# MengLing-L/distributed_plonk

Measured on AMD Instinct MI355X. Metric: constraints/sec = n / proof time (verified five-round proof, dispatcher2.rs:192-713; BN254 PLONK), higher is better.
Workload: dtype u32x8 Montgomery (256-bit Fr/Fq)

## Files before the change

distributed_plonk_amd/csrc/ntt_engine.hip:

```cpp
#include <algorithm>
#include <cstdlib>
#include <cstring>

#include "constants.h"
#include "ntt_kernels.hpp"
#include "plonk_internal.hpp"

static int ilog2(uint64_t x) { int l = 0; while (((uint64_t)1 << (l + 1)) <= x) l++; return l; }
static_assert(NTT_LOG_RMAX == 9, "NttTables::max_log_r defaults to NTT_LOG_RMAX");

const FrParams& fr_params(int curve) { return curve == PLONK_BN254 ? BN254_FR_PARAMS : BLS12_381_FR_PARAMS; }

static Fr host_pow2k(const Fr& a, int k, const FrParams& P) {
    Fr r = a;
    for (int i = 0; i < k; i++) r = fp_sqr(r, P);
    return r;
}

static int upload_powers(F29** d_out, const Fr& base, size_t count, const Fr& first, const FrParams& P, hipStream_t stream) {
    std::vector<F29> h(count);
    Fr r261;
    for (int i = 0; i < 8; i++) r261.l[i] = P.one[i];
    for (int i = 0; i < 5; i++) r261 = fp_add(r261, r261, P);
    const Fr k_mont = fp_to_mont(r261, P);
// ... 33 lines not shown
        if ((rc = upload_powers(&T.tw_small[d], host_pow2k(w[d], T.two_adicity - NTT_LOG_RMAX, P),
                                (size_t)1 << (NTT_LOG_RMAX - 1), one, P, stream))) return rc;
        {
            const size_t cnt = (size_t)1 << (NTT_LOG_RMAX - 1);
            std::vector<F29S> h(cnt);
            const Fr base = host_pow2k(w[d], T.two_adicity - NTT_LOG_RMAX, P);
            Fr acc = one;
            for (size_t i = 0; i < cnt; i++) { h[i] = f29_shoup_from_mont256(acc, P); acc = fp_mul(acc, base, P); }
            HIP_TRY(hipMalloc((void**)&T.tw_shoup[d], cnt * sizeof(F29S)));
            HIP_TRY(hipMemcpyAsync(T.tw_shoup[d], h.data(), cnt * sizeof(F29S), hipMemcpyHostToDevice, stream));
            HIP_TRY(hipStreamSynchronize(stream));
        }
        if ((rc = upload_powers(&T.g_lo[d], g[d], nt, one, P, stream))) return rc;
        if ((rc = upload_powers(&T.g_hi[d], host_pow2k(g[d], T.lt, P), nt, one, P, stream))) return rc;
    }
    T.use_shoup = getenv("PLONK_NTT_NO_SHOUP") == nullptr;
    Fr two = fp_add(one, one, P), half = fp_inv(two, P);
    T.h_pow2_inv.resize(T.two_adicity + 1);
    Fr acc = one;
    for (int k = 0; k <= T.two_adicity; k++) { T.h_pow2_inv[k] = acc; acc = fp_mul(acc, half, P); }
    return PLONK_OK;
}

void ntt_tables_trim(NttTables& T) {
    for (auto& kv : T.tw_lo_scaled) (void)hipFree(kv.second);
    T.tw_lo_scaled.clear();
    for (auto& kv : T.planes) (void)hipFree(kv.second);
    T.planes.clear();
    for (auto& kv : T.rowtabs) (void)hipFree(kv.second);
    T.rowtabs.clear();
    for (auto& kv : T.shift_sets) { (void)hipFree(kv.second.planes); (void)hipFree(kv.second.rowtabs); (void)hipFree(kv.second.foldc); }
    T.shift_sets.clear();
    T.plane_bytes = 0;
    for (auto& kv : T.quot_inv_xm1) (void)hipFree(kv.second);
    T.quot_inv_xm1.clear();
    for (auto& kv : T.pow_tabs) (void)hipFree(kv.second);
    T.pow_tabs.clear();
    T.pow_order.clear();
}

void ntt_tables_destroy(NttTables& T) {
    for (int d = 0; d < 2; d++) {
        (void)hipFree(T.tw_shoup[d]); T.tw_shoup[d] = nullptr;
        (void)hipFree(T.tw_small[d]); (void)hipFree(T.tw_lo[d]); (void)hipFree(T.tw_hi[d]); (void)hipFree(T.g_lo[d]); (void)hipFree(T.g_hi[d]);
        T.tw_small[d] = T.tw_lo[d] = T.tw_hi[d] = T.g_lo[d] = T.g_hi[d] = nullptr;
    }
    for (auto& kv : T.tw_lo_scaled) (void)hipFree(kv.second);
    T.tw_lo_scaled.clear();
    for (auto& kv : T.planes) (void)hipFree(kv.second);
    T.planes.clear();
    for (auto& kv : T.rowtabs) (void)hipFree(kv.second);
    T.rowtabs.clear();
    for (auto& kv : T.shift_sets) { (void)hipFree(kv.second.planes); (void)hipFree(kv.second.rowtabs); (void)hipFree(kv.second.foldc); }
    T.shift_sets.clear();
    T.plane_bytes = 0;
    if (T.quot_x_lo) { (void)hipFree(T.quot_x_lo); T.quot_x_lo = nullptr; }
    for (auto& kv : T.quot_inv_xm1) (void)hipFree(kv.second);
    T.quot_inv_xm1.clear();
    for (auto& kv : T.pow_tabs) (void)hipFree(kv.second);
    T.pow_tabs.clear();
    T.pow_order.clear();
}

static int get_scaled_lo(NttTables& T, int log_m, F29** out, hipStream_t stream) {
    auto it = T.tw_lo_scaled.find(log_m);
    if (it != T.tw_lo_scaled.end()) { *out = it->second; return PLONK_OK; }
    F29* d = nullptr;
    int rc = upload_powers(&d, T.h_root[1], (size_t)1 << T.lt, T.h_pow2_inv[log_m], T.fp, stream);
    if (rc) return rc;
    T.tw_lo_scaled[log_m] = d;
    *out = d;
    return PLONK_OK;
}

static void plane_fallback_notice(const char* why, size_t bytes) {
    static bool said = false;
// ... 53 lines not shown
    hipError_t e = hipGetLastError();
    if (e != hipSuccess) { (void)hipFree(d); return plonk_fail(PLONK_ERR_HIP, "ntt_gen_epi_plane launch: %s", hipGetErrorString(e)); }
    T.planes[key] = d;
    T.plane_bytes += bytes;
    *out = d;
    return PLONK_OK;
}

static int get_rowtab(NttTables& T, int log_r1, int log_w, F29** out, hipStream_t stream) {
    const uint64_t key = ((uint64_t)log_r1 << 8) | (uint64_t)log_w;
    auto it = T.rowtabs.find(key);
    if (it != T.rowtabs.end()) { *out = it->second; return PLONK_OK; }
    const uint32_t* g_l = T.curve == PLONK_BN254 ? BN254_FR_GENERATOR_MONT : BLS12_381_FR_GENERATOR_MONT;
    Fr base = fp_from_limbs<8>(g_l);
    for (int i = 0; i < log_r1; i++) base = fp_sqr(base, T.fp);
    F29* d = nullptr;
    int rc = upload_powers(&d, base, (size_t)1 << log_w, fp_one(T.fp), T.fp, stream);
    if (rc) return rc;
    T.rowtabs[key] = d;
    *out = d;
    return PLONK_OK;
}

static void host_powers_const(std::vector<F29>& h, const Fr& base, size_t count, const FrParams& P) {
    Fr r261;
    for (int i = 0; i < 8; i++) r261.l[i] = P.one[i];
    for (int i = 0; i < 5; i++) r261 = fp_add(r261, r261, P);
    const Fr k_mont = fp_to_mont(r261, P);
    Fr acc = fp_one(P);
    for (size_t i = 0; i < count; i++) {
        h.push_back(f29_from_sat(fp_from_mont(fp_mul(acc, k_mont, P), P)));
        acc = fp_mul(acc, base, P);
    }
}

static int get_shift_set(NttTables& T, const Fr& h, int L, uint64_t B, int w0, int NP, const NttTables::ShiftSet** out, hipStream_t stream) {
    const FrParams& P = T.fp;
    const int logB = ilog2(B);
    std::string key((const char*)h.l, 32);
    key.push_back((char)L); key.push_back((char)logB); key.push_back((char)w0);
    auto it = T.shift_sets.find(key);
    if (it != T.shift_sets.end()) { *out = &it->second; return PLONK_OK; }
    if (L + logB > T.two_adicity) return plonk_fail(PLONK_ERR_DOMAIN, "coset classes: 2^%d points exceed the two-adicity", L + logB);
    const uint64_t M = (uint64_t)1 << L, R1 = (uint64_t)1 << w0, r1 = M >> w0;
    NttTables::ShiftSet set;
    set.bytes = NP > 1 ? (size_t)(B * M) * sizeof(Fr) : 0;
    if (T.plane_bytes + set.bytes > T.plane_budget && !T.shift_sets.empty()) {
        HIP_TRY(hipStreamSynchronize(stream));
        for (auto& kv : T.shift_sets) {
            (void)hipFree(kv.second.planes); (void)hipFree(kv.second.rowtabs); (void)hipFree(kv.second.foldc);
            T.plane_bytes -= kv.second.bytes;
        }
        T.shift_sets.clear();
    }
    if (T.plane_bytes + set.bytes > T.plane_budget)
        return plonk_fail(PLONK_ERR_HIP, "coset classes: %zu bytes of first-pass planes exceed the plane budget (%zu of %zu in use)", set.bytes,
                          T.plane_bytes, T.plane_budget);
    const Fr wB = host_pow2k(T.h_root[0], T.two_adicity - (L + logB), P);
    std::vector<F29> h_row, h_fold;
    h_row.reserve(B * R1); h_fold.reserve(B * NTT_MAX_FOLD);
    std::vector<Fr> hq(B);
    Fr acc = h;
    for (uint64_t q = 0; q < B; q++) { hq[q] = acc; acc = fp_mul(acc, wB, P); }
    for (uint64_t q = 0; q < B; q++) {
        host_powers_const(h_row, host_pow2k(hq[q], L - w0, P), R1, P);
        host_powers_const(h_fold, host_pow2k(hq[q], L, P), NTT_MAX_FOLD, P);
    }
    struct Guard {
        NttTables::ShiftSet* s; F29* extra = nullptr; bool armed = true;
        ~Guard() { if (armed) { (void)hipFree(s->planes); (void)hipFree(s->rowtabs); (void)hipFree(s->foldc); } (void)hipFree(extra); }
    } guard{&set};
    HIP_TRY(hipMalloc((void**)&set.rowtabs, h_row.size() * sizeof(F29)));
    HIP_TRY(hipMalloc((void**)&set.foldc, h_fold.size() * sizeof(F29)));
    HIP_TRY(hipMemcpyAsync(set.rowtabs, h_row.data(), h_row.size() * sizeof(F29), hipMemcpyHostToDevice, stream));
    HIP_TRY(hipMemcpyAsync(set.foldc, h_fold.data(), h_fold.size() * sizeof(F29), hipMemcpyHostToDevice, stream));
    HIP_TRY(hipStreamSynchronize(stream));
    if (NP > 1) {
        if (hipMalloc((void**)&set.planes, set.bytes) != hipSuccess) {
            (void)hipGetLastError();
            set.planes = nullptr;
            return plonk_fail(PLONK_ERR_HIP, "coset classes: out of memory for %zu bytes of first-pass planes", set.bytes);
        }
        const size_t n_hi = (size_t)std::max<uint64_t>(1, r1 >> 10);
        std::vector<F29> h_pw;
        h_pw.reserve(B * (1024 + n_hi));
        for (uint64_t q = 0; q < B; q++) {
            host_powers_const(h_pw, hq[q], 1024, P);
            host_powers_const(h_pw, host_pow2k(hq[q], 10, P), n_hi, P);
        }
        F29* d_pw = nullptr;
        HIP_TRY(hipMalloc((void**)&d_pw, h_pw.size() * sizeof(F29)));
        guard.extra = d_pw;
        HIP_TRY(hipMemcpyAsync(d_pw, h_pw.data(), h_pw.size() * sizeof(F29), hipMemcpyHostToDevice, stream));
        for (uint64_t q = 0; q < B; q++) {
            const F29* lo = d_pw + q * (1024 + n_hi);
            ProfScope ps("ntt_gen_shift_plane", stream);
            hipLaunchKernelGGL(ntt_gen_shift_plane_kernel, dim3((uint32_t)((M + 255) / 256)), dim3(256), 0, stream, set.planes + q * M, M, r1, T.tw_lo[0],
                               T.tw_hi[0], (uint32_t)T.lt, (uint32_t)(T.two_adicity - L), lo, lo + 1024, T.fp29);
// ... 44 lines not shown
    if (s.kind == 1 || s.kind == 2) {
        o.lo = T.g_lo[s.kind - 1];
        o.hi = T.g_hi[s.kind - 1];
    } else {
        const int d = s.kind - 3;
        o.lo = T.tw_lo[d];
        o.hi = T.tw_hi[d];
        const int sh = T.two_adicity - s.log_order;
        aq <<= sh; a0 <<= sh; bq <<= sh; b0 <<= sh;
    }
    o.aq = aq; o.a0 = a0; o.bq = bq; o.b0 = b0;
    return o;
}

static int ntt_ept() {
    static const int ept = [] {
        const char* e = getenv("PLONK_NTT_EPT");
        const int v = e ? atoi(e) : 4;
        return (v == 4 || v == 2) ? v : (e ? 8 : 4);
    }();
    return ept;
}

template <int LOG_R, int EPT, bool SWZ = false, bool SHOUP = false>
static hipError_t launch_one_e(const NttPassParams& P, uint64_t grid, uint32_t threads, size_t lds, hipStream_t stream) {
    static DeviceOnce attr;
    hipError_t e = attr.run([] { return hipFuncSetAttribute(reinterpret_cast<const void*>(&ntt_pass_kernel<LOG_R, EPT, SWZ, SHOUP>),
                                                           hipFuncAttributeMaxDynamicSharedMemorySize, 160 * 1024); });
    if (e != hipSuccess) return e;
    hipLaunchKernelGGL((ntt_pass_kernel<LOG_R, EPT, SWZ, SHOUP>), dim3((uint32_t)grid), dim3(threads), lds, stream, P);
    return hipGetLastError();
}
static bool swizzle_on() {
    static const bool on = getenv("PLONK_NTT_NO_SWIZZLE") == nullptr;
    return on;
}
template <int LOG_R>
static hipError_t launch_one(const NttPassParams& P, uint64_t grid, uint32_t threads, size_t lds, hipStream_t stream) {
    if constexpr (LOG_R >= 5) {
        if (ntt_ept() == 4 && P.log_t == 3 && P.tile_pitch == 8 && swizzle_on()) {
            if (P.tw_shoup != nullptr) return launch_one_e<LOG_R, 4, true, true>(P, grid, threads, lds, stream);
            return launch_one_e<LOG_R, 4, true>(P, grid, threads, lds, stream);
        }
    }
    if (ntt_ept() == 4) return launch_one_e<LOG_R, 4>(P, grid, threads, lds, stream);
    if (ntt_ept() == 2) return launch_one_e<LOG_R, 2>(P, grid, threads, lds, stream);
    return launch_one_e<LOG_R, 8>(P, grid, threads, lds, stream);
}

static hipError_t launch_pass(int log_r, const NttPassParams& P, uint64_t grid, uint32_t threads, size_t lds, hipStream_t s) {
    switch (log_r) {
        case 1: return launch_one<1>(P, grid, threads, lds, s);
        case 2: return launch_one<2>(P, grid, threads, lds, s);
        case 3: return launch_one<3>(P, grid, threads, lds, s);
        case 4: return launch_one<4>(P, grid, threads, lds, s);
        case 5: return launch_one<5>(P, grid, threads, lds, s);
        case 6: return launch_one<6>(P, grid, threads, lds, s);
        case 7: return launch_one<7>(P, grid, threads, lds, s);
        case 8: return launch_one<8>(P, grid, threads, lds, s);
        case 9: return launch_one<9>(P, grid, threads, lds, s);
    }
    return hipErrorInvalidValue;
}
// ... 109 lines not shown
                P.plane_rp = r_p;
            }
            avail = interleaved ? Bt : r_p;
            int lt = std::min(pref_log_t(w), ilog2(avail));
            const uint64_t Tt = (uint64_t)1 << lt;
            P.log_t = lt;
            if (!interleaved) {
                P.n0 = r_p / Tt; P.n1 = M / r_prev;
                P.ls0 = Tt; P.ls1 = r_prev; P.ls2 = M; P.l_astride = r_p; P.l_tstride = 1;
                P.bs0 = Tt; P.bs1 = 0; P.tb = 1;
                P.qs0 = 0; P.qs1 = 0; P.qs2 = 1; P.tq = 0;
                P.pa = r_p; P.ps0 = Tt; P.ps1 = 0; P.pt = 1;
                grid = Bt * P.n1 * P.n0;
            } else {
                P.n0 = Bt / Tt; P.n1 = r_p;
                P.ls0 = Tt; P.ls1 = Bt; P.ls2 = r_prev * Bt; P.l_astride = r_p * Bt; P.l_tstride = 1;
                P.bs0 = 0; P.bs1 = 1; P.tb = 0;
                P.qs0 = Tt; P.qs1 = 0; P.qs2 = 0; P.tq = 1;
                P.pa = r_p; P.ps0 = 0; P.ps1 = 1; P.pt = 0;
                grid = (M / r_prev) * P.n1 * P.n0;
            }
            P.ss0 = P.ls0; P.ss1 = P.ls1; P.ss2 = P.ls2; P.s_istride = P.l_astride; P.s_tstride = 1;
            P.tile_pitch = (uint32_t)Tt;
        } else {
            P.out = c.out;
            P.kstride = M >> w;
            if (sset != nullptr && NP >= 2 && n_cls >= 2) {
                avail = Bt;
                int lt = std::min(pref_log_t(w), ilog2(avail));
                const uint64_t Tt = (uint64_t)1 << lt;
                P.log_t = lt;
                P.n0 = Bt / Tt; P.n1 = M >> w;
                P.ls0 = Tt * M; P.ls1 = R; P.ls2 = 0; P.l_astride = 1; P.l_tstride = M; P.load_a_fast = 1;
                P.qs0 = Tt; P.tq = 1;
                P.ms0 = 0; P.tk = 0;
                P.rev_ndig = NP - 1;
                for (int d = 0; d < NP - 1; d++) P.rev_w[d] = widths[d];
                P.rev_shift0 = 0;
                grid = P.n0 * P.n1;
            } else if (!interleaved && NP >= 2) {
                const uint64_t R1 = (uint64_t)1 << widths[0], r1 = M >> widths[0];
                avail = R1;
                int lt = std::min(pref_log_t(w), ilog2(avail));
                const uint64_t Tt = (uint64_t)1 << lt;
                P.log_t = lt;
                P.n0 = R1 / Tt; P.n1 = (M >> w) / R1;
// ... 37 lines not shown
            if (c.inverse && NP == 1) { P.scale_const_enabled = 1; P.scale_const = f29_const_from_mont256(T.h_pow2_inv[L], T.fp); }
            if (epi_plane != nullptr && (!need_q_const || coset_folded || sset != nullptr)) {
                P.epi_plane = epi_plane;
                P.epi_qstride = M * n_cls;
            } else {
                P.epi = make_scale(T, c.epi, c.q_offset);
            }
            P.tile_pitch = (uint32_t)((uint64_t)1 << P.log_t);
        }
        if (p == 0 && !coset_folded) P.pro = make_scale(T, c.pro, c.q_offset);
        const uint64_t Tt = (uint64_t)1 << P.log_t;
        const uint32_t ept = (R >= (uint64_t)ntt_ept()) ? (uint32_t)ntt_ept() : (uint32_t)R;
        const uint32_t threads = (uint32_t)(R * Tt / ept);
        if (threads > 1024) return plonk_fail(PLONK_ERR_ARG, "ntt_run: tile of %llu x %llu needs %u lanes", (unsigned long long)R, (unsigned long long)Tt, threads);
        const size_t lds = (size_t)9 * R * P.tile_pitch * 4 + std::max<size_t>(R / 2, 1) * 36;
        if (grid == 0 || grid > 0x7fffffffull) return plonk_fail(PLONK_ERR_ARG, "ntt_run: grid %llu out of range", (unsigned long long)grid);
        static const char* const kNames[10] = {"", "ntt_pass_kernel<1>", "ntt_pass_kernel<2>", "ntt_pass_kernel<3>", "ntt_pass_kernel<4>",
                                               "ntt_pass_kernel<5>", "ntt_pass_kernel<6>", "ntt_pass_kernel<7>", "ntt_pass_kernel<8>",
                                               "ntt_pass_kernel<9>"};
        hipError_t e;
        {
            ProfScope ps_all("ntt_pass_kernel", stream);
            ProfScope ps_w(kNames[w], stream);
            e = launch_pass(w, P, grid, threads, lds, stream);
        }
        if (e != hipSuccess) return plonk_fail(PLONK_ERR_HIP, "ntt pass launch (log_r=%d, grid=%llu, threads=%u, lds=%zu): %s", w,
                                               (unsigned long long)grid, threads, lds, hipGetErrorString(e));
        r_prev = r_p;
    }
    return PLONK_OK;
}

__global__ void __launch_bounds__(256) transpose_fr_kernel(const Fr* __restrict__ in, Fr* __restrict__ out, uint64_t rows, uint64_t cols) {
    __shared__ uint4 tile[16][16 * 2 + 1];
    const uint64_t tiles_c = (cols + 15) / 16;
    const uint64_t tr = blockIdx.x / tiles_c, tc = blockIdx.x % tiles_c;
    const uint32_t ly = threadIdx.x / 16, lx = threadIdx.x % 16;
    uint64_t r = tr * 16 + ly, cc = tc * 16 + lx;
    if (r < rows && cc < cols) {
        const uint4* src = reinterpret_cast<const uint4*>(in + r * cols + cc);
        tile[ly][2 * lx] = src[0];
        tile[ly][2 * lx + 1] = src[1];
    }
    __syncthreads();
    uint64_t orow = tc * 16 + ly, ocol = tr * 16 + lx;
    if (orow < cols && ocol < rows) {
// ... 17 lines not shown
```

distributed_plonk_amd/csrc/ntt_kernels.hpp:

```cpp
#pragma once
#include "fp.hpp"
#include "fp29.hpp"

typedef Fp<8> Fr;
typedef FpParams<8> FrParams;

#define NTT_LOG_RMAX 9
#define NTT_MAX_PASSES 4
#define NTT_MAX_FOLD 8

struct TwoLevelScale {
    const F29* lo;
    const F29* hi;
    uint64_t aq, a0, bq, b0;
    uint32_t lt;
    uint32_t enabled;
};

struct NttPassParams {
    const Fr* in;
    Fr* out;
    F29Params fp;
    const F29* tw_small;
    const F29S* tw_shoup;
// ... 17 lines not shown
    uint32_t rev_ndig;
    uint32_t rev_w[NTT_MAX_PASSES];
    uint32_t rev_shift0;
    uint64_t oq, ok;
    int32_t split_log;
    uint64_t split_blk;
    const Fr* tw_plane;
    uint64_t plane_rp;
    const F29* pro_rowtab;
    uint64_t rowtab_qstride;
    uint64_t plane_qstride;
    uint64_t in_len;
    uint64_t fold_m;
    uint32_t nfold;
    const F29* fold_c;
    uint32_t cls_log;
    uint64_t in_row_pitch;
    const Fr* epi_plane;
    uint64_t epi_qstride;
    uint32_t scale_const_enabled;
    F29 scale_const;
    TwoLevelScale pro;
    TwoLevelScale epi;
};

__device__ __forceinline__ Fr load_fr(const Fr* p) {
    const uint4* q = reinterpret_cast<const uint4*>(p);
    uint4 a = q[0], b = q[1];
    Fr r;
    r.l[0] = a.x; r.l[1] = a.y; r.l[2] = a.z; r.l[3] = a.w;
    r.l[4] = b.x; r.l[5] = b.y; r.l[6] = b.z; r.l[7] = b.w;
    return r;
}
__device__ __forceinline__ void store_fr(Fr* p, const Fr& v) {
    uint4* q = reinterpret_cast<uint4*>(p);
    q[0] = make_uint4(v.l[0], v.l[1], v.l[2], v.l[3]);
    q[1] = make_uint4(v.l[4], v.l[5], v.l[6], v.l[7]);
}
__device__ __forceinline__ F29 load_f29(const F29* p) {
    F29 r;
    const uint32_t* q = reinterpret_cast<const uint32_t*>(p);
#pragma unroll
    for (int i = 0; i < 9; i++) r.l[i] = q[i];
    return r;
}
__device__ __forceinline__ F29 params_one(const F29Params& P) {
// ... 25 lines not shown
    __device__ __forceinline__ void put(uint32_t idx, const F29& v) const {
#pragma unroll
        for (int l = 0; l < 9; l++) base[l * plane + idx] = v.l[l];
    }
};

template <bool SWZ> __device__ __forceinline__ uint32_t sw_fold(uint32_t row) {
    if (!SWZ) return 0;
    uint32_t y = row >> 2;
    y ^= y >> 4;
    y ^= y >> 2;
    return y & 3;
}

template <int LOG_R>
__device__ __forceinline__ void shoup_tw_load(const F29S* __restrict__ tab, uint32_t e, uint32_t* cw) {
    const uint4* src = reinterpret_cast<const uint4*>(tab + ((size_t)e << (NTT_LOG_RMAX - LOG_R)));
#pragma unroll
    for (int j = 0; j < 5; j++) {
        const uint4 d = src[j];
        cw[4 * j] = d.x; cw[4 * j + 1] = d.y; cw[4 * j + 2] = d.z; cw[4 * j + 3] = d.w;
    }
}
template <int LOG_R, int K, bool FIRST, bool SHOUP>
__device__ __forceinline__ void ntt_butterflies(F29 (&v)[1 << K], int s0, uint32_t lo, const uint32_t* tw_lds, const F29S* __restrict__ tw_shoup,
                                                const F29Params& fp) {
    constexpr int R = 1 << LOG_R;
    constexpr int RADIX = 1 << K;
    constexpr int TWN = (R / 2 > 0) ? R / 2 : 1;
    const uint32_t h = 1u << s0;
#pragma unroll
    for (int ds = 0; ds < K; ds++) {
        const int span = 1 << ds;
#pragma unroll
        for (int k = 0; k < RADIX; k++) {
            if (k & span) continue;
            const int kk = k & (span - 1);
            F29 tt;
            const F29 x = v[k];
            if (FIRST && kk == 0 && ds <= 1) {
                tt = v[k + span];
                v[k] = f29_add(x, tt);
                v[k + span] = (ds == 0) ? f29_sub2p(x, tt, fp) : f29_sub4p(x, tt, fp);
            } else {
                const uint32_t e = (lo + kk * h) << (LOG_R - s0 - ds - 1);
                if constexpr (SHOUP) {
                    uint32_t cw[20];
                    shoup_tw_load<LOG_R>(tw_shoup, e, cw);
                    tt = f29_mul_shoup(v[k + span], cw, cw + 9, fp);
                    v[k] = f29_add(x, tt);
                    v[k + span] = f29_sub4p(x, tt, fp);
                } else {
                    F29 tw;
#pragma unroll
                    for (int l = 0; l < 9; l++) tw.l[l] = tw_lds[l * TWN + e];
                    tt = f29_mul(v[k + span], tw, fp);
                    v[k] = f29_add(x, tt);
                    v[k + span] = f29_sub2p(x, tt, fp);
                }
            }
            __builtin_amdgcn_sched_barrier(0);
        }
        if (ds == 1 || ds == K - 1) {
#pragma unroll
            for (int k = 0; k < RADIX; k++) f29_norm(v[k]);
        }
    }
}

template <int LOG_R, int K, int EPT, bool FIRST, bool SWZ, bool SHOUP>
__device__ __forceinline__ void ntt_step(const LdsTile& tile, const uint32_t* tw_lds, const F29S* __restrict__ tw_shoup, int s0, uint32_t w, uint32_t t,
                                         uint32_t pitch, const F29Params& fp) {
    constexpr int R = 1 << LOG_R;
    constexpr int RADIX = 1 << K;
    constexpr int NG = EPT / RADIX;
    constexpr int GROUPS_PER_STRIDE = R / EPT;
    const uint32_t h = 1u << s0;
#pragma unroll
    for (int g = 0; g < NG; g++) {
        const uint32_t G = w + g * GROUPS_PER_STRIDE;
        const uint32_t lo = G & (h - 1), hi = G >> s0;
        const uint32_t a0 = (hi << (s0 + K)) | lo;
        F29 v[RADIX];
        const uint32_t fa = sw_fold<SWZ>(a0);
#pragma unroll
        for (int k = 0; k < RADIX; k++) v[k] = tile.get(((a0 + k * h) ^ fa ^ sw_fold<SWZ>(k * h)) * pitch + t);
        ntt_butterflies<LOG_R, K, FIRST, SHOUP>(v, s0, lo, tw_lds, tw_shoup, fp);
#pragma unroll
        for (int k = 0; k < RADIX; k++) tile.put(((a0 + k * h) ^ fa ^ sw_fold<SWZ>(k * h)) * pitch + t, v[k]);
    }
}

#ifdef NTT_XLANE
template <int LOG_R, bool SWZ, bool SHOUP>
__device__ __forceinline__ void ntt_steps0123_xlane(const LdsTile& tile, const uint32_t* tw_lds, const F29S* __restrict__ tw_shoup, uint32_t w, uint32_t t,
                                                    uint32_t pitch, const F29Params& fp) {
    const uint32_t we = (w & ~7u) | ((w >> 1) & 3u) | ((w & 1u) << 2);
    F29 v[4];
    {
        const uint32_t a0 = we << 2, fa = sw_fold<SWZ>(a0);
#pragma unroll
        for (int k = 0; k < 4; k++) v[k] = tile.get(((a0 + k) ^ fa ^ sw_fold<SWZ>(k)) * pitch + t);
    }
    ntt_butterflies<LOG_R, 2, true, SHOUP>(v, 0, 0, tw_lds, tw_shoup, fp);
#pragma unroll
    for (int l = 0; l < 9; l++) {
        auto r01 = __builtin_amdgcn_permlane16_swap(v[0].l[l], v[1].l[l], false, false);
        auto r23 = __builtin_amdgcn_permlane16_swap(v[2].l[l], v[3].l[l], false, false);
        v[0].l[l] = r01[0]; v[1].l[l] = r01[1]; v[2].l[l] = r23[0]; v[3].l[l] = r23[1];
    }
#pragma unroll
    for (int l = 0; l < 9; l++) {
        auto r02 = __builtin_amdgcn_permlane32_swap(v[0].l[l], v[2].l[l], false, false);
        auto r13 = __builtin_amdgcn_permlane32_swap(v[1].l[l], v[3].l[l], false, false);
        v[0].l[l] = r02[0]; v[2].l[l] = r02[1]; v[1].l[l] = r13[0]; v[3].l[l] = r13[1];
    }
    const uint32_t lo = we & 3u, hi = we >> 2;
    ntt_butterflies<LOG_R, 2, false, SHOUP>(v, 2, lo, tw_lds, tw_shoup, fp);
    const uint32_t a0 = (hi << 4) | lo, fa = sw_fold<SWZ>(a0);
#pragma unroll
    for (int k = 0; k < 4; k++) tile.put(((a0 + k * 4) ^ fa ^ sw_fold<SWZ>(k * 4)) * pitch + t, v[k]);
}
#endif

template <int LOG_R, int EPT_REQ, bool SWZ = false, bool SHOUP = false>
__global__ void __launch_bounds__(EPT_REQ <= 4 ? 1024 : 512) ntt_pass_kernel(const NttPassParams P) {
    constexpr int R = 1 << LOG_R;
    constexpr int EPT = (R >= EPT_REQ) ? EPT_REQ : R;
    constexpr int KMAX = (EPT == 8) ? 3 : (EPT == 4) ? 2 : (EPT == 2 ? 1 : 1);
    constexpr int TWN = (R / 2 > 0) ? R / 2 : 1;
    extern __shared__ __attribute__((aligned(16))) uint32_t smem[];
    const uint32_t LOG_T = SWZ ? 3u : P.log_t;
    const uint32_t T = 1u << LOG_T;
    const uint32_t pitch = SWZ ? 8u : P.tile_pitch;
    const uint32_t plane = R * pitch;
    const uint32_t nthreads = (R * T) / EPT;
    const uint32_t u = threadIdx.x;
    LdsTile tile{smem, plane};
    uint32_t* tw_lds = smem + 9 * plane;

    const uint64_t ti = blockIdx.x;
    const uint64_t x0 = ti % P.n0, x12 = ti / P.n0, x1 = x12 % P.n1, x2 = x12 / P.n1;
    const uint64_t lbase = x0 * P.ls0 + x1 * P.ls1 + x2 * P.ls2;
    const uint64_t b0 = x0 * P.bs0 + x1 * P.bs1;
    const uint64_t q0 = x0 * P.qs0 + x1 * P.qs1 + x2 * P.qs2;

    if constexpr (!SHOUP) {
        for (uint32_t e = u; e < TWN; e += nthreads) {
            const F29 tw = load_f29(P.tw_small + ((uint64_t)e << (NTT_LOG_RMAX - LOG_R)));
#pragma unroll
            for (int l = 0; l < 9; l++) tw_lds[l * TWN + e] = tw.l[l];
// ... 10 lines not shown
        const uint64_t arr = q0 + (uint64_t)t * P.tq;
        const uint64_t cls = arr & (((uint64_t)1 << P.cls_log) - 1);
        if (P.in_len != 0) {
            const uint64_t pos = (uint64_t)a * P.pa + x0 * P.ps0 + x1 * P.ps1 + (uint64_t)t * P.pt;
            const Fr* src = P.in + (arr >> P.cls_log) * P.in_row_pitch;
            if (pos < P.in_len) {
                v = f29_from_sat(load_fr(src + pos));
            } else {
#pragma unroll
                for (int l = 0; l < 9; l++) v.l[l] = 0;
            }
            if (P.nfold > 1 && pos + P.fold_m < P.in_len) {
                const F29* fc = P.fold_c + NTT_MAX_FOLD * cls;
                for (uint32_t uu = 1; uu < P.nfold; uu++) {
                    const uint64_t j = pos + (uint64_t)uu * P.fold_m;
                    if (j < P.in_len) v = f29_add(v, f29_mul(f29_from_sat(load_fr(src + j)), load_f29(fc + uu), P.fp));
                    if (uu == 3) f29_norm(v);
                }
                f29_norm(v);
            }
        } else {
            v = f29_from_sat(load_fr(P.in + lbase + (uint64_t)a * P.l_astride + (uint64_t)t * P.l_tstride));
        }
        if (P.pro_rowtab != nullptr) {
            v = f29_mul(v, load_f29(P.pro_rowtab + cls * P.rowtab_qstride + a), P.fp);
        } else if (P.pro.enabled) {
            const uint64_t pos = (uint64_t)a * P.pa + x0 * P.ps0 + x1 * P.ps1 + (uint64_t)t * P.pt;
            const F29 s = two_level(P.pro, pos, arr, P.fp);
            v = f29_mul(v, s, P.fp);
        }
        const uint32_t row = brev(a, LOG_R);
        tile.put((row ^ sw_fold<SWZ>(row)) * pitch + t, v);
    }
    __syncthreads();

    {
        const uint32_t t = u & (T - 1), w = u >> LOG_T;
        constexpr int KREM = LOG_R % KMAX;
        constexpr int SFULL = LOG_R - KREM;
        if constexpr (R <= EPT) {
            ntt_step<LOG_R, LOG_R, EPT, true, SWZ, SHOUP>(tile, tw_lds, P.tw_shoup, 0, w, t, pitch, P.fp);
            __syncthreads();
        } else {
            if constexpr (SFULL > 0) {
#ifdef NTT_XLANE
                constexpr bool XL = SWZ && EPT == 4 && LOG_R >= 7;
#else
                constexpr bool XL = false;
#endif
                if constexpr (XL) {
#ifdef NTT_XLANE
                    ntt_steps0123_xlane<LOG_R, SWZ, SHOUP>(tile, tw_lds, P.tw_shoup, w, t, pitch, P.fp);
#endif
                } else {
                    ntt_step<LOG_R, KMAX, EPT, true, SWZ, SHOUP>(tile, tw_lds, P.tw_shoup, 0, w, t, pitch, P.fp);
                }
                __syncthreads();
#pragma unroll 1
                for (int s = XL ? 2 * KMAX : KMAX; s < SFULL; s += KMAX) {
                    ntt_step<LOG_R, KMAX, EPT, false, SWZ, SHOUP>(tile, tw_lds, P.tw_shoup, s, w, t, pitch, P.fp);
                    __syncthreads();
                }
            }
            if constexpr (KREM != 0) {
                ntt_step<LOG_R, KREM, EPT, SFULL == 0, SWZ, SHOUP>(tile, tw_lds, P.tw_shoup, SFULL, w, t, pitch, P.fp);
                __syncthreads();
            }
        }
    }

    uint64_t m0 = 0;
    if (P.is_last) {
        m0 = x0 * P.ms0;
        uint32_t total = 0;
        for (uint32_t d = 0; d < P.rev_ndig; d++) total += P.rev_w[d];
        uint32_t sh = P.rev_shift0, consumed = 0;
        for (uint32_t d = 0; d < P.rev_ndig; d++) {
            consumed += P.rev_w[d];
            const uint64_t dig = (x1 >> (total - consumed)) & (((uint64_t)1 << P.rev_w[d]) - 1);
            m0 |= dig << sh;
            sh += P.rev_w[d];
        }
    }
    const uint64_t sbase = x0 * P.ss0 + x1 * P.ss1 + x2 * P.ss2;
#pragma unroll
    for (int i = 0; i < EPT; i++) {
        const uint32_t e = u + i * nthreads;
        const uint32_t t = e & (T - 1), idx = e >> LOG_T;
// ... 90 lines not shown
```

distributed_plonk_amd/csrc/plonk_api.hip:

```cpp
#include <cstdarg>
#include <cstring>
#include <map>
#include <memory>
#include <mutex>
#include <algorithm>
#include <vector>

#include "constants.h"
#include "ec.hpp"
#include "plonk_internal.hpp"
#include "pairing.hpp"


static thread_local char g_err[512] = {0};
char* plonk_last_error_buf() { return g_err; }
int plonk_fail(int code, const char* fmt, ...) {
    va_list ap;
    va_start(ap, fmt);
    vsnprintf(g_err, sizeof g_err, fmt, ap);
    va_end(ap);
    return code;
}
extern "C" const char* plonk_last_error(void) { return g_err; }

// ... 203 lines not shown
    if (!strcmp(key, "msm_window")) { ctx->msm_window = (int)value; return PLONK_OK; }
    if (!strcmp(key, "comm_check_order")) { g_comm_check = value ? 1 : 0; return PLONK_OK; }
    if (!strcmp(key, "check_bases")) { ctx->check_bases = value ? 1 : 0; return PLONK_OK; }
    if (!strcmp(key, "msm_precompute")) { ctx->msm_precompute = (int)value; return PLONK_OK; }
    if (!strcmp(key, "msm_table_c")) {
        if (value != 0 && (value < 4 || value > 21)) return plonk_fail(PLONK_ERR_ARG, "msm_table_c = %lld (0 or 4..21)", (long long)value);
        ctx->msm_table_c = (int)value;
        return PLONK_OK;
    }
    if (!strcmp(key, "msm_table_sets")) { ctx->msm_table_sets = (int)value; return PLONK_OK; }
    if (!strcmp(key, "msm_table_budget_mib")) { ctx->msm_table_budget = (size_t)value << 20; return PLONK_OK; }
    if (!strcmp(key, "ntt_max_log_r")) { ctx->tables.max_log_r = (int)value; return PLONK_OK; }
    if (!strcmp(key, "msm_batch_max")) { ctx->msm_ws.batch_max = (int)value; return PLONK_OK; }
    if (!strcmp(key, "msm_fused_order")) { ctx->msm_ws.fused_order = value < 0 ? 0 : (value > 2 ? 2 : (int)value); return PLONK_OK; }
    if (!strcmp(key, "msm_fused_y3")) { ctx->msm_ws.fused_y3 = value ? 1 : 0; return PLONK_OK; }
    if (!strcmp(key, "msm_sort_stage_cap")) { ctx->msm_ws.sort_stage_cap = (int)std::max<int64_t>(0, value); return PLONK_OK; }
    if (!strcmp(key, "msm_sort_slice_index")) { ctx->msm_ws.sort_slice_index = value ? 1 : 0; return PLONK_OK; }
    if (!strcmp(key, "msm_acc_persist")) { ctx->msm_ws.acc_persist = (int)std::max<int64_t>(-65536, std::min<int64_t>(value, 8)); return PLONK_OK; }
    if (!strcmp(key, "msm_reduce_grid")) { ctx->msm_ws.reduce_grid = value ? 1 : 0; return PLONK_OK; }
    if (!strcmp(key, "ntt_shoup")) {
        ctx->tables.use_shoup = value != 0;
        return PLONK_OK;
    }
    if (!strcmp(key, "ntt_plane_budget")) {
        ctx->tables.plane_budget = value < 0 ? NTT_PLANE_BUDGET_DEFAULT : (size_t)value;
        return PLONK_OK;
    }
    if (!strcmp(key, "quotient_fuse")) { ctx->tables.quotient_fuse = (int)value; return PLONK_OK; }
    if (!strcmp(key, "msm_slice_log")) { ctx->msm_ws.slice_log = (int)value; return PLONK_OK; }
    return plonk_fail(PLONK_ERR_ARG, "plonk_set_option: unknown key %s", key);
}

extern "C" int plonk_msm_plan(plonk_ctx* ctx, size_t n, int K, int32_t* out, int n_out) {
    CHECK_CTX(ctx);
    return msm_plan_query(ctx->curve, n, K, ctx->msm_ws, ctx->msm_window, ctx->msm_table, out, n_out);
}

extern "C" int plonk_last_kernel_ms(plonk_ctx* ctx, double* out_ms) {
    CHECK_CTX(ctx);
    if (!out_ms || !ctx->ev_valid) return plonk_fail(PLONK_ERR_STATE, "no timed call yet");
    HIP_TRY(hipEventSynchronize(ctx->ev1));
    float ms = 0;
    HIP_TRY(hipEventElapsedTime(&ms, ctx->ev0, ctx->ev1));
    *out_ms = ms;
    return PLONK_OK;
}
// ... 1181 lines not shown
```

distributed_plonk_amd/csrc/plonk_internal.hpp:

```cpp
#pragma once
#include <hip/hip_runtime.h>
#include <stdint.h>
#include <stdio.h>
#include <mutex>
#include <string>
#include <unordered_map>
#include <vector>

#include "fp.hpp"
#include "fp29.hpp"
#include "../../include/plonk_hip.h"

typedef Fp<8> Fr;
typedef FpParams<8> FrParams;

#define HIP_TRY(expr)                                                                          \
    do {                                                                                       \
        hipError_t _e = (expr);                                                                \
        if (_e != hipSuccess) {                                                                \
            snprintf(plonk_last_error_buf(), 512, "%s:%d: %s -> %s", __FILE__, __LINE__, #expr, \
                     hipGetErrorString(_e));                                                   \
            return PLONK_ERR_HIP;                                                              \
        }                                                                                      \
    } while (0)
// ... 7 lines not shown
        int dev = 0;
        hipError_t e = hipGetDevice(&dev);
        if (e != hipSuccess) return e;
        const uint64_t bit = dev >= 0 && dev < 64 ? (uint64_t)1 << dev : 0;
        if (bit && (__atomic_load_n(&done, __ATOMIC_ACQUIRE) & bit)) return hipSuccess;
        e = set();
        if (e == hipSuccess && bit) __atomic_fetch_or(&done, bit, __ATOMIC_RELEASE);
        return e;
    }
};

struct KernelProfiler {
    std::mutex mu;
    bool enabled = false;
    struct Rec { const char* name; hipEvent_t a, b; };
    std::vector<Rec> pending;
    std::unordered_map<std::string, std::pair<double, uint64_t>> totals;
    void resolve();
    void reset();
};
KernelProfiler& kernel_profiler();
struct ProfScope {
    const char* name; hipStream_t stream; hipEvent_t a = nullptr, b = nullptr; bool on;
    ProfScope(const char* n, hipStream_t s) : name(n), stream(s), on(kernel_profiler().enabled) {
        if (on) { (void)hipEventCreate(&a); (void)hipEventCreate(&b); (void)hipEventRecord(a, stream); }
    }
    ~ProfScope() {
        if (on) {
            (void)hipEventRecord(b, stream);
            std::lock_guard<std::mutex> g(kernel_profiler().mu);
            kernel_profiler().pending.push_back({name, a, b});
        }
    }
};

constexpr size_t NTT_PLANE_BUDGET_DEFAULT = (size_t)48 << 30;
struct NttTables {
    int curve = 0;
    FrParams fp;
    F29Params fp29;
    int two_adicity = 0;
    int lt = 0;
    F29* tw_small[2] = {nullptr, nullptr};
    F29S* tw_shoup[2] = {nullptr, nullptr};
    bool use_shoup = false;
    F29* tw_lo[2] = {nullptr, nullptr};
    F29* tw_hi[2] = {nullptr, nullptr};
    F29* g_lo[2] = {nullptr, nullptr};
    F29* g_hi[2] = {nullptr, nullptr};
    std::unordered_map<int, F29*> tw_lo_scaled;
    std::unordered_map<uint64_t, Fr*> planes;
    std::unordered_map<uint64_t, F29*> rowtabs;
    struct ShiftSet {
        Fr* planes = nullptr;
        F29* rowtabs = nullptr;
        F29* foldc = nullptr;
        size_t bytes = 0;
    };
    std::unordered_map<std::string, ShiftSet> shift_sets;
    size_t plane_bytes = 0;
    size_t plane_budget = NTT_PLANE_BUDGET_DEFAULT;
    F29* quot_x_lo = nullptr;
    std::unordered_map<int, Fr*> quot_inv_xm1;
    std::unordered_map<std::string, F29*> pow_tabs;
    std::vector<std::string> pow_order;
    int max_log_r = 9;
    int quotient_fuse = 6;
    std::vector<Fr> h_pow2_inv;
    Fr h_root[2];
};

enum NttLayout { NTT_CONTIGUOUS = 0, NTT_INTERLEAVED = 1 };

struct ScaleSpec {
    int kind = 0;
    uint64_t aq = 0, a0 = 0, bq = 0, b0 = 0;
    int log_order = 0;
};

// ... 129 lines not shown
```

Measured before the change: 21.24 million.

## Fold coset prologue scaling into first-pass NTT twiddles

Adds per-coset twiddle tables that multiply the coset shift into every butterfly twiddle of the first NTT pass. The separate per-element prologue multiply by a row table is dropped. The first stage now also uses twiddle products instead of the twiddle-free first butterflies. This removes one Montgomery multiply and one global table load per element, but adds multiplies in the first stage, larger twiddle tables (per class) read from global memory, and host-side table construction. It is enabled by default only for the swizzled Shoup shape with log_r>=5, and it disables the cross-lane step variant on that path.

```diff
diff --git a/distributed_plonk_amd/csrc/ntt_engine.hip b/distributed_plonk_amd/csrc/ntt_engine.hip
--- a/distributed_plonk_amd/csrc/ntt_engine.hip
+++ b/distributed_plonk_amd/csrc/ntt_engine.hip
@@ -79,6 +79,11 @@
     return PLONK_OK;
 }
 
+static void shift_set_free(NttTables::ShiftSet& s) {
+    (void)hipFree(s.planes); (void)hipFree(s.rowtabs); (void)hipFree(s.foldc); (void)hipFree(s.ctw);
+    s.planes = nullptr; s.rowtabs = nullptr; s.foldc = nullptr; s.ctw = nullptr;
+}
+
 void ntt_tables_trim(NttTables& T) {
     for (auto& kv : T.tw_lo_scaled) (void)hipFree(kv.second);
     T.tw_lo_scaled.clear();
@@ -86,7 +91,9 @@
     T.planes.clear();
     for (auto& kv : T.rowtabs) (void)hipFree(kv.second);
     T.rowtabs.clear();
-    for (auto& kv : T.shift_sets) { (void)hipFree(kv.second.planes); (void)hipFree(kv.second.rowtabs); (void)hipFree(kv.second.foldc); }
+    for (auto& kv : T.ctw_tabs) (void)hipFree(kv.second);
+    T.ctw_tabs.clear();
+    for (auto& kv : T.shift_sets) shift_set_free(kv.second);
     T.shift_sets.clear();
     T.plane_bytes = 0;
     for (auto& kv : T.quot_inv_xm1) (void)hipFree(kv.second);
@@ -108,7 +115,9 @@
     T.planes.clear();
     for (auto& kv : T.rowtabs) (void)hipFree(kv.second);
     T.rowtabs.clear();
-    for (auto& kv : T.shift_sets) { (void)hipFree(kv.second.planes); (void)hipFree(kv.second.rowtabs); (void)hipFree(kv.second.foldc); }
+    for (auto& kv : T.ctw_tabs) (void)hipFree(kv.second);
+    T.ctw_tabs.clear();
+    for (auto& kv : T.shift_sets) shift_set_free(kv.second);
     T.shift_sets.clear();
     T.plane_bytes = 0;
     if (T.quot_x_lo) { (void)hipFree(T.quot_x_lo); T.quot_x_lo = nullptr; }
@@ -208,6 +217,30 @@
     return PLONK_OK;
 }
 
+static void host_coset_twiddles(std::vector<F29S>& h, const Fr& s, int w, const NttTables& T) {
+    for (int sg = 0; sg < w; sg++) {
+        const Fr root = host_pow2k(T.h_root[0], T.two_adicity - (sg + 1), T.fp);
+        Fr acc = host_pow2k(s, w - sg - 1, T.fp);
+        for (uint32_t j = 0; j < (1u << sg); j++) { h.push_back(f29_shoup_from_mont256(acc, T.fp)); acc = fp_mul(acc, root, T.fp); }
+    }
+}
+
+static int get_coset_tw(NttTables& T, int log_r1, int log_w, const F29S** out, hipStream_t stream) {
+    const uint64_t key = ((uint64_t)log_r1 << 8) | (uint64_t)log_w;
+    auto it = T.ctw_tabs.find(key);
+    if (it != T.ctw_tabs.end()) { *out = it->second; return PLONK_OK; }
+    const uint32_t* g_l = T.curve == PLONK_BN254 ? BN254_FR_GENERATOR_MONT : BLS12_381_FR_GENERATOR_MONT;
+    std::vector<F29S> h;
+    host_coset_twiddles(h, host_pow2k(fp_from_limbs<8>(g_l), log_r1, T.fp), log_w, T);
+    F29S* d = nullptr;
+    HIP_TRY(hipMalloc((void**)&d, h.size() * sizeof(F29S)));
+    T.ctw_tabs[key] = d;
+    HIP_TRY(hipMemcpyAsync(d, h.data(), h.size() * sizeof(F29S), hipMemcpyHostToDevice, stream));
+    HIP_TRY(hipStreamSynchronize(stream));
+    *out = d;
+    return PLONK_OK;
+}
+
 static void host_powers_const(std::vector<F29>& h, const Fr& base, size_t count, const FrParams& P) {
     Fr r261;
     for (int i = 0; i < 8; i++) r261.l[i] = P.one[i];
@@ -234,8 +267,8 @@
     if (T.plane_bytes + set.bytes > T.plane_budget && !T.shift_sets.empty()) {
         HIP_TRY(hipStreamSynchronize(stream));
         for (auto& kv : T.shift_sets) {
-            (void)hipFree(kv.second.planes); (void)hipFree(kv.second.rowtabs); (void)hipFree(kv.second.foldc);
             T.plane_bytes -= kv.second.bytes;
+            shift_set_free(kv.second);
         }
         T.shift_sets.clear();
     }
@@ -254,12 +287,19 @@
     }
     struct Guard {
         NttTables::ShiftSet* s; F29* extra = nullptr; bool armed = true;
-        ~Guard() { if (armed) { (void)hipFree(s->planes); (void)hipFree(s->rowtabs); (void)hipFree(s->foldc); } (void)hipFree(extra); }
+        ~Guard() { if (armed) shift_set_free(*s); (void)hipFree(extra); }
     } guard{&set};
     HIP_TRY(hipMalloc((void**)&set.rowtabs, h_row.size() * sizeof(F29)));
     HIP_TRY(hipMalloc((void**)&set.foldc, h_fold.size() * sizeof(F29)));
     HIP_TRY(hipMemcpyAsync(set.rowtabs, h_row.data(), h_row.size() * sizeof(F29), hipMemcpyHostToDevice, stream));
     HIP_TRY(hipMemcpyAsync(set.foldc, h_fold.data(), h_fold.size() * sizeof(F29), hipMemcpyHostToDevice, stream));
+    std::vector<F29S> h_ctw;
+    if (NP > 1 && w0 >= 5) {
+        h_ctw.reserve(B * (R1 - 1));
+        for (uint64_t q = 0; q < B; q++) host_coset_twiddles(h_ctw, host_pow2k(hq[q], L - w0, P), w0, T);
+        HIP_TRY(hipMalloc((void**)&set.ctw, h_ctw.size() * sizeof(F29S)));
+        HIP_TRY(hipMemcpyAsync(set.ctw, h_ctw.data(), h_ctw.size() * sizeof(F29S), hipMemcpyHostToDevice, stream));
+    }
     HIP_TRY(hipStreamSynchronize(stream));
     if (NP > 1) {
         if (hipMalloc((void**)&set.planes, set.bytes) != hipSuccess) {
@@ -350,23 +390,27 @@
     return ept;
 }
 
-template <int LOG_R, int EPT, bool SWZ = false, bool SHOUP = false>
+template <int LOG_R, int EPT, bool SWZ = false, bool SHOUP = false, bool CTW = false>
 static hipError_t launch_one_e(const NttPassParams& P, uint64_t grid, uint32_t threads, size_t lds, hipStream_t stream) {
     static DeviceOnce attr;
-    hipError_t e = attr.run([] { return hipFuncSetAttribute(reinterpret_cast<const void*>(&ntt_pass_kernel<LOG_R, EPT, SWZ, SHOUP>),
+    hipError_t e = attr.run([] { return hipFuncSetAttribute(reinterpret_cast<const void*>(&ntt_pass_kernel<LOG_R, EPT, SWZ, SHOUP, CTW>),
                                                            hipFuncAttributeMaxDynamicSharedMemorySize, 160 * 1024); });
     if (e != hipSuccess) return e;
-    hipLaunchKernelGGL((ntt_pass_kernel<LOG_R, EPT, SWZ, SHOUP>), dim3((uint32_t)grid), dim3(threads), lds, stream, P);
+    hipLaunchKernelGGL((ntt_pass_kernel<LOG_R, EPT, SWZ, SHOUP, CTW>), dim3((uint32_t)grid), dim3(threads), lds, stream, P);
     return hipGetLastError();
 }
 static bool swizzle_on() {
     static const bool on = getenv("PLONK_NTT_NO_SWIZZLE") == nullptr;
     return on;
+}
+static bool swizzled_shoup_shape(const NttTables& T, int log_r, const NttPassParams& P) {
+    return log_r >= 5 && T.use_shoup && ntt_ept() == 4 && P.log_t == 3 && P.tile_pitch == 8 && swizzle_on();
 }
 template <int LOG_R>
 static hipError_t launch_one(const NttPassParams& P, uint64_t grid, uint32_t threads, size_t lds, hipStream_t stream) {
     if constexpr (LOG_R >= 5) {
         if (ntt_ept() == 4 && P.log_t == 3 && P.tile_pitch == 8 && swizzle_on()) {
+            if (P.tw_shoup != nullptr && P.ctw != nullptr) return launch_one_e<LOG_R, 4, true, true, true>(P, grid, threads, lds, stream);
             if (P.tw_shoup != nullptr) return launch_one_e<LOG_R, 4, true, true>(P, grid, threads, lds, stream);
             return launch_one_e<LOG_R, 4, true>(P, grid, threads, lds, stream);
         }
@@ -522,6 +566,16 @@
             }
             P.ss0 = P.ls0; P.ss1 = P.ls1; P.ss2 = P.ls2; P.s_istride = P.l_astride; P.s_tstride = 1;
             P.tile_pitch = (uint32_t)Tt;
+            if (p == 0 && P.pro_rowtab != nullptr && T.coset_twiddles && !interleaved && swizzled_shoup_shape(T, w, P)) {
+                if (sset != nullptr) {
+                    P.ctw = sset->ctw;
+                    P.ctw_qstride = R - 1;
+                } else {
+                    int rc = get_coset_tw(T, log_b0 + ilog2(r_p), w, &P.ctw, stream);
+                    if (rc) return rc;
+                }
+                if (P.ctw != nullptr) P.pro_rowtab = nullptr;
+            }
         } else {
             P.out = c.out;
             P.kstride = M >> w;
@@ -605,6 +659,7 @@
         {
             ProfScope ps_all("ntt_pass_kernel", stream);
             ProfScope ps_w(kNames[w], stream);
+            ProfScope ps_ctw("ntt_pass_coset_tw", stream, P.ctw != nullptr);
             e = launch_pass(w, P, grid, threads, lds, stream);
         }
         if (e != hipSuccess) return plonk_fail(PLONK_ERR_HIP, "ntt pass launch (log_r=%d, grid=%llu, threads=%u, lds=%zu): %s", w,
diff --git a/distributed_plonk_amd/csrc/ntt_kernels.hpp b/distributed_plonk_amd/csrc/ntt_kernels.hpp
--- a/distributed_plonk_amd/csrc/ntt_kernels.hpp
+++ b/distributed_plonk_amd/csrc/ntt_kernels.hpp
@@ -63,6 +63,8 @@
     F29 scale_const;
     TwoLevelScale pro;
     TwoLevelScale epi;
+    const F29S* ctw;
+    uint64_t ctw_qstride;
 };
 
 __device__ __forceinline__ Fr load_fr(const Fr* p) {
@@ -134,12 +136,13 @@
         cw[4 * j] = d.x; cw[4 * j + 1] = d.y; cw[4 * j + 2] = d.z; cw[4 * j + 3] = d.w;
     }
 }
-template <int LOG_R, int K, bool FIRST, bool SHOUP>
+template <int LOG_R, int K, bool FIRST, bool SHOUP, bool CTW = false>
 __device__ __forceinline__ void ntt_butterflies(F29 (&v)[1 << K], int s0, uint32_t lo, const uint32_t* tw_lds, const F29S* __restrict__ tw_shoup,
                                                 const F29Params& fp) {
     constexpr int R = 1 << LOG_R;
     constexpr int RADIX = 1 << K;
     constexpr int TWN = (R / 2 > 0) ? R / 2 : 1;
+    static_assert(!CTW || (SHOUP && !FIRST), "coset twiddles: every stage carries a prepared-constant product");
     const uint32_t h = 1u << s0;
 #pragma unroll
     for (int ds = 0; ds < K; ds++) {
@@ -158,7 +161,8 @@
                 const uint32_t e = (lo + kk * h) << (LOG_R - s0 - ds - 1);
                 if constexpr (SHOUP) {
                     uint32_t cw[20];
-                    shoup_tw_load<LOG_R>(tw_shoup, e, cw);
+                    if constexpr (CTW) shoup_tw_load<NTT_LOG_RMAX>(tw_shoup, (h << ds) - 1 + lo + kk * h, cw);
+                    else shoup_tw_load<LOG_R>(tw_shoup, e, cw);
                     tt = f29_mul_shoup(v[k + span], cw, cw + 9, fp);
                     v[k] = f29_add(x, tt);
                     v[k + span] = f29_sub4p(x, tt, fp);
@@ -180,7 +184,7 @@
     }
 }
 
-template <int LOG_R, int K, int EPT, bool FIRST, bool SWZ, bool SHOUP>
+template <int LOG_R, int K, int EPT, bool FIRST, bool SWZ, bool SHOUP, bool CTW = false>
 __device__ __forceinline__ void ntt_step(const LdsTile& tile, const uint32_t* tw_lds, const F29S* __restrict__ tw_shoup, int s0, uint32_t w, uint32_t t,
                                          uint32_t pitch, const F29Params& fp) {
     constexpr int R = 1 << LOG_R;
@@ -197,7 +201,7 @@
         const uint32_t fa = sw_fold<SWZ>(a0);
 #pragma unroll
         for (int k = 0; k < RADIX; k++) v[k] = tile.get(((a0 + k * h) ^ fa ^ sw_fold<SWZ>(k * h)) * pitch + t);
-        ntt_butterflies<LOG_R, K, FIRST, SHOUP>(v, s0, lo, tw_lds, tw_shoup, fp);
+        ntt_butterflies<LOG_R, K, FIRST, SHOUP, CTW>(v, s0, lo, tw_lds, tw_shoup, fp);
 #pragma unroll
         for (int k = 0; k < RADIX; k++) tile.put(((a0 + k * h) ^ fa ^ sw_fold<SWZ>(k * h)) * pitch + t, v[k]);
     }
@@ -235,10 +239,11 @@
 }
 #endif
 
-template <int LOG_R, int EPT_REQ, bool SWZ = false, bool SHOUP = false>
+template <int LOG_R, int EPT_REQ, bool SWZ = false, bool SHOUP = false, bool CTW = false>
 __global__ void __launch_bounds__(EPT_REQ <= 4 ? 1024 : 512) ntt_pass_kernel(const NttPassParams P) {
     constexpr int R = 1 << LOG_R;
     constexpr int EPT = (R >= EPT_REQ) ? EPT_REQ : R;
+    static_assert(!CTW || (SWZ && SHOUP && R > EPT), "coset twiddles are built for the swizzled prepared-constant shape");
     constexpr int KMAX = (EPT == 8) ? 3 : (EPT == 4) ? 2 : (EPT == 2 ? 1 : 1);
     constexpr int TWN = (R / 2 > 0) ? R / 2 : 1;
     extern __shared__ __attribute__((aligned(16))) uint32_t smem[];
@@ -295,12 +300,14 @@
         } else {
             v = f29_from_sat(load_fr(P.in + lbase + (uint64_t)a * P.l_astride + (uint64_t)t * P.l_tstride));
         }
-        if (P.pro_rowtab != nullptr) {
-            v = f29_mul(v, load_f29(P.pro_rowtab + cls * P.rowtab_qstride + a), P.fp);
-        } else if (P.pro.enabled) {
-            const uint64_t pos = (uint64_t)a * P.pa + x0 * P.ps0 + x1 * P.ps1 + (uint64_t)t * P.pt;
-            const F29 s = two_level(P.pro, pos, arr, P.fp);
-            v = f29_mul(v, s, P.fp);
+        if constexpr (!CTW) {
+            if (P.pro_rowtab != nullptr) {
+                v = f29_mul(v, load_f29(P.pro_rowtab + cls * P.rowtab_qstride + a), P.fp);
+            } else if (P.pro.enabled) {
+                const uint64_t pos = (uint64_t)a * P.pa + x0 * P.ps0 + x1 * P.ps1 + (uint64_t)t * P.pt;
+                const F29 s = two_level(P.pro, pos, arr, P.fp);
+                v = f29_mul(v, s, P.fp);
+            }
         }
         const uint32_t row = brev(a, LOG_R);
         tile.put((row ^ sw_fold<SWZ>(row)) * pitch + t, v);
@@ -311,32 +318,33 @@
         const uint32_t t = u & (T - 1), w = u >> LOG_T;
         constexpr int KREM = LOG_R % KMAX;
         constexpr int SFULL = LOG_R - KREM;
+        const F29S* const tws = CTW ? P.ctw + (q0 & (((uint64_t)1 << P.cls_log) - 1)) * P.ctw_qstride : P.tw_shoup;
         if constexpr (R <= EPT) {
-            ntt_step<LOG_R, LOG_R, EPT, true, SWZ, SHOUP>(tile, tw_lds, P.tw_shoup, 0, w, t, pitch, P.fp);
+            ntt_step<LOG_R, LOG_R, EPT, true, SWZ, SHOUP>(tile, tw_lds, tws, 0, w, t, pitch, P.fp);
             __syncthreads();
         } else {
             if constexpr (SFULL > 0) {
 #ifdef NTT_XLANE
-                constexpr bool XL = SWZ && EPT == 4 && LOG_R >= 7;
+                constexpr bool XL = !CTW && SWZ && EPT == 4 && LOG_R >= 7;
 #else
                 constexpr bool XL = false;
 #endif
                 if constexpr (XL) {
 #ifdef NTT_XLANE
-                    ntt_steps0123_xlane<LOG_R, SWZ, SHOUP>(tile, tw_lds, P.tw_shoup, w, t, pitch, P.fp);
+                    ntt_steps0123_xlane<LOG_R, SWZ, SHOUP>(tile, tw_lds, tws, w, t, pitch, P.fp);
 #endif
                 } else {
-                    ntt_step<LOG_R, KMAX, EPT, true, SWZ, SHOUP>(tile, tw_lds, P.tw_shoup, 0, w, t, pitch, P.fp);
+                    ntt_step<LOG_R, KMAX, EPT, !CTW, SWZ, SHOUP, CTW>(tile, tw_lds, tws, 0, w, t, pitch, P.fp);
                 }
                 __syncthreads();
 #pragma unroll 1
                 for (int s = XL ? 2 * KMAX : KMAX; s < SFULL; s += KMAX) {
-                    ntt_step<LOG_R, KMAX, EPT, false, SWZ, SHOUP>(tile, tw_lds, P.tw_shoup, s, w, t, pitch, P.fp);
+                    ntt_step<LOG_R, KMAX, EPT, false, SWZ, SHOUP, CTW>(tile, tw_lds, tws, s, w, t, pitch, P.fp);
                     __syncthreads();
                 }
             }
             if constexpr (KREM != 0) {
-                ntt_step<LOG_R, KREM, EPT, SFULL == 0, SWZ, SHOUP>(tile, tw_lds, P.tw_shoup, SFULL, w, t, pitch, P.fp);
+                ntt_step<LOG_R, KREM, EPT, SFULL == 0 && !CTW, SWZ, SHOUP, CTW>(tile, tw_lds, tws, SFULL, w, t, pitch, P.fp);
                 __syncthreads();
             }
         }
diff --git a/distributed_plonk_amd/csrc/plonk_api.hip b/distributed_plonk_amd/csrc/plonk_api.hip
--- a/distributed_plonk_amd/csrc/plonk_api.hip
+++ b/distributed_plonk_amd/csrc/plonk_api.hip
@@ -249,6 +249,7 @@
         ctx->tables.use_shoup = value != 0;
         return PLONK_OK;
     }
+    if (!strcmp(key, "ntt_coset_twiddles")) { ctx->tables.coset_twiddles = value != 0; return PLONK_OK; }
     if (!strcmp(key, "ntt_plane_budget")) {
         ctx->tables.plane_budget = value < 0 ? NTT_PLANE_BUDGET_DEFAULT : (size_t)value;
         return PLONK_OK;
diff --git a/distributed_plonk_amd/csrc/plonk_internal.hpp b/distributed_plonk_amd/csrc/plonk_internal.hpp
--- a/distributed_plonk_amd/csrc/plonk_internal.hpp
+++ b/distributed_plonk_amd/csrc/plonk_internal.hpp
@@ -53,7 +53,7 @@
 KernelProfiler& kernel_profiler();
 struct ProfScope {
     const char* name; hipStream_t stream; hipEvent_t a = nullptr, b = nullptr; bool on;
-    ProfScope(const char* n, hipStream_t s) : name(n), stream(s), on(kernel_profiler().enabled) {
+    ProfScope(const char* n, hipStream_t s, bool wanted = true) : name(n), stream(s), on(wanted && kernel_profiler().enabled) {
         if (on) { (void)hipEventCreate(&a); (void)hipEventCreate(&b); (void)hipEventRecord(a, stream); }
     }
     ~ProfScope() {
@@ -82,10 +82,13 @@
     std::unordered_map<int, F29*> tw_lo_scaled;
     std::unordered_map<uint64_t, Fr*> planes;
     std::unordered_map<uint64_t, F29*> rowtabs;
+    std::unordered_map<uint64_t, F29S*> ctw_tabs;
+    bool coset_twiddles = true;
     struct ShiftSet {
         Fr* planes = nullptr;
         F29* rowtabs = nullptr;
         F29* foldc = nullptr;
+        F29S* ctw = nullptr;
         size_t bytes = 0;
     };
     std::unordered_map<std::string, ShiftSet> shift_sets;
```

Result: faster. 21.58 million, median of 6 (+1.6%).
